# JosephCatrambone/aruco3

Hardware: NVIDIA B200
Metric: frames_per_sec_1080p_batch256 (higher is better)
Workload: dtype u8/u32 integer pixels, f32/f64 decode

## Files before the change

aruco3_b200/csrc/k3_contours.cu:

```cuda
#include <cooperative_groups.h>
#include <cooperative_groups/scan.h>
#include <cub/device/device_radix_sort.cuh>

#include <stdio.h>
#include <stdlib.h>

#include <algorithm>
#include <optional>

#include "a3_internal.h"

namespace a3 {
namespace {

namespace cg = cooperative_groups;

constexpr int kDx[8] = {-1, -1, 0, 1, 1, 1, 0, -1};
constexpr int kDy[8] = {0, -1, -1, -1, 0, 1, 1, 1};

struct StepTables {
    uint16_t fwd[8][512];
    uint16_t bwd[8][512];
};

// ... 16 lines not shown
                }
                const uint16_t e = (uint16_t)(d | (((examined >> 0) & 1u) << 3) | (((examined >> 4) & 1u) << 4) | ((kDx[d] + 1) << 5) |
                                              ((kDy[d] + 1) << 7) | (((d + 4) & 7) << 10));
                (back ? t.bwd : t.fwd)[state][hood] = e;
            }
        }
}

__device__ __forceinline__ int ddx(int d) { return (d >= 3 && d <= 5) ? 1 : ((d == 2 || d == 6) ? 0 : -1); }
__device__ __forceinline__ int ddy(int d) { return (d >= 1 && d <= 3) ? -1 : ((d == 0 || d == 4) ? 0 : 1); }

struct Geo {
    const uint32_t *planes;
    uint32_t n, w, h, wpr, Hp;
    size_t frame_words;
};

__device__ __forceinline__ uint32_t hood9(const uint32_t *plane, uint32_t Hp, int x, int y) {
    const int o = x + 31;
    const uint32_t *p = plane + ((uint32_t)(o >> 5) * Hp + (uint32_t)y);
    const int sh = o & 31;
    uint32_t t = __ldg(p) >> sh, m = __ldg(p + 1) >> sh, b = __ldg(p + 2) >> sh;
    if (sh > 29) {
        const uint32_t *q = p + Hp;
        t |= __ldg(q) << (32 - sh); m |= __ldg(q + 1) << (32 - sh); b |= __ldg(q + 2) << (32 - sh);
    }
    return (t & 7u) | ((m & 7u) << 3) | ((b & 7u) << 6);
}
__device__ __forceinline__ uint32_t ring_of(uint32_t hood) {
    const uint32_t t = hood & 7u, m = (hood >> 3) & 7u, b = hood >> 6;
    return (m & 1u) | ((t & 1u) << 1) | ((t & 2u) << 1) | ((t & 4u) << 1) | ((m & 4u) << 2) | ((b & 4u) << 3) | ((b & 2u) << 5) | ((b & 1u) << 7);
}

struct Window {
    const uint32_t *plane;
    uint32_t Hp;
    int kc, yg;
    uint32_t t, m, b;
    uint32_t t2, m2, b2;
    uint32_t v2;
};
__device__ __forceinline__ void win_load(Window &w, int x, int y) {
    w.kc = (x + 31) >> 5; w.yg = y;
    const uint32_t *p = w.plane + (size_t)w.kc * w.Hp + y;
    w.t = __ldg(p); w.m = __ldg(p + 1); w.b = __ldg(p + 2);
    w.v2 = 0;
}
__device__ __forceinline__ uint32_t win_hood(Window &w, int x) {
    const int sh = (x + 31) & 31;
    uint32_t t = w.t >> sh, m = w.m >> sh, b = w.b >> sh;
    if (sh > 29) {
        if (w.v2 != 7u) {
            const uint32_t *q = w.plane + (size_t)(w.kc + 1) * w.Hp + w.yg;
            if (!(w.v2 & 1u)) w.t2 = __ldg(q);
            if (!(w.v2 & 2u)) w.m2 = __ldg(q + 1);
            if (!(w.v2 & 4u)) w.b2 = __ldg(q + 2);
            w.v2 = 7u;
        }
        t |= w.t2 << (32 - sh); m |= w.m2 << (32 - sh); b |= w.b2 << (32 - sh);
    }
    return (t & 7u) | ((m & 7u) << 3) | ((b & 7u) << 6);
}
__device__ __forceinline__ void win_move(Window &w, int x, int y) {
    const int kc = (x + 31) >> 5, dy = y - w.yg;
    if (kc != w.kc) {
        if (dy == 0 && kc == w.kc + 1 && w.v2 == 7u) {
            w.t = w.t2; w.m = w.m2; w.b = w.b2; w.v2 = 0; w.kc = kc;
        } else if (dy == 0 && kc == w.kc - 1) {
            w.t2 = w.t; w.m2 = w.m; w.b2 = w.b; w.v2 = 7u; w.kc = kc;
            const uint32_t *p = w.plane + (size_t)kc * w.Hp + y;
            w.t = __ldg(p); w.m = __ldg(p + 1); w.b = __ldg(p + 2);
        } else {
            win_load(w, x, y);
        }
    } else if (dy > 0) {
        w.t = w.m; w.m = w.b; w.b = __ldg(w.plane + (size_t)kc * w.Hp + y + 2);
        w.t2 = w.m2; w.m2 = w.b2; w.v2 >>= 1;
        w.yg = y;
    } else if (dy < 0) {
        w.b = w.m; w.m = w.t; w.t = __ldg(w.plane + (size_t)kc * w.Hp + y);
        w.b2 = w.m2; w.m2 = w.t2; w.v2 = (w.v2 << 1) & 7u;
        w.yg = y;
    }
}

constexpr uint32_t kBudget = 48;
constexpr uint32_t kSeg = 64;
static_assert(kBudget < kSeg, "borders finished inside the budget must fit one emit segment");
struct Ckpt { uint32_t walker, pos, xy, state; };
constexpr uint32_t kCkptBackward = 0x80000000u;

enum { kDead = 0, kSurvivor = 1, kUndecided = 2 };
constexpr uint32_t kNumWalkers = 0;
constexpr uint32_t kNumLong = 1;
constexpr uint32_t kOverflow = 2;
constexpr uint32_t kNumCands = 3;
constexpr uint32_t kNumCkpts = 4;
constexpr uint32_t kSpecFail = 5;
constexpr uint32_t kNumRelays = 6;
constexpr uint32_t kMaxFrameLong = 7;

struct Lists {
    unsigned long long *cands;
    uint32_t cands_cap;
    unsigned long long *walkers;
    unsigned long long *long_keys;
    uint32_t *long_n;
    uint32_t *counters;
    uint32_t *long_slot;
    uint32_t *walker_slot;
    Ckpt *ckpts;
    uint32_t ckpt_cap;
    unsigned long long *long_points;
    uint32_t walkers_cap, long_cap;
    uint32_t *frame_contours;
    unsigned long long *frame_points;
    uint32_t *frame_flags;
    uint32_t *long_off_slot;
    uint32_t frame_cap;
    uint32_t *frame_long_count;
    unsigned long long *frame_keys;
    uint32_t *frame_slots;
    uint2 *relays;
    struct Seg *segs;
    uint32_t *relay_base;
    unsigned long long *seg_owner;
    struct Jump *jumps;
    unsigned long long *anchor_owner;
    uint32_t jump_hops;
    uint32_t relay_cap;
    uint32_t relay_shift, nrr;
};
struct __align__(16) Seg {
    uint32_t next;
    uint32_t len;
    uint32_t cand;
    uint32_t cand_pos;
    uint32_t min_pix;
    uint32_t slot;
    uint32_t off;
    uint32_t state;
};
struct __align__(16) Jump {
    uint32_t dest;
    uint32_t len;
    uint32_t cand;
    uint32_t cand_off;
    uint32_t min_pix;
    uint32_t min_idx;
    uint32_t pad0, pad1;
};
constexpr uint32_t kNone = 0xffffffffu;
constexpr uint32_t kRelayFlag = 0x80000000u;


__device__ __forceinline__ uint32_t hood2(const uint32_t *plane, uint32_t Hp, int o, int y) {
    const uint32_t *p = plane + ((uint32_t)(o >> 5) * Hp + (uint32_t)y);
    const int sh = o & 31;
    uint32_t t = __ldg(p), m = __ldg(p + 1), b = __ldg(p + 2), t2 = 0, m2 = 0, b2 = 0;
    if (sh > 29) {
        const uint32_t *q = p + Hp;
        t2 = __ldg(q); m2 = __ldg(q + 1); b2 = __ldg(q + 2);
    }
    t = __funnelshift_r(t, t2, sh); m = __funnelshift_r(m, m2, sh); b = __funnelshift_r(b, b2, sh);
    return ((t << 1) & 0x00eu) | ((m << 4) & 0x070u) | ((b << 7) & 0x380u);
}

template <bool relay_on>
__device__ int walk_border(const uint32_t *plane, const Geo &g, const uint16_t (*fwd)[512], const uint16_t (*bwd)[512], int sx, int sy, int kind,
                           uint32_t budget, uint32_t &n, bool &first_pixel, uint32_t rmask) {
    const int w = (int)g.w, o_max = w + 30;
    const uint32_t start_pix = (uint32_t)(sy * w + sx);
    const uint32_t me = (start_pix << 1) | (uint32_t)kind;
    const uint32_t nb0 = ring_of(hood9(plane, g.Hp, sx, sy));
    const int adj = kind ? 4 : 0;
    int pred = -1;
    for (int k = 0; k < 8; k++) {
        const int d = (adj + k) & 7;
        if ((nb0 >> d) & 1) { pred = d; break; }
    }
    n = 1;
    first_pixel = true;
    if (pred < 0) return (kind == 0 || sx == 0) ? kSurvivor : kDead;
    if (relay_on && ((uint32_t)sy & rmask) == 0u) return kDead;
    uint32_t min_pix = start_pix, pix = start_pix, state_off;
    int o = sx + 31, y = sy;
    if (kind) {
        state_off = (uint32_t)pred << 10;
        n = 0;
    } else {
        o += ddx(pred); y += ddy(pred); pix = (uint32_t)(y * w + o - 31); state_off = (uint32_t)((pred + 4) & 7) << 10;
    }
    const unsigned char *lut = reinterpret_cast<const unsigned char *>(kind ? &fwd[0][0] : &bwd[0][0]);
    const uint32_t tw = (me + 1u) >> 1, te = me >> 1, pred_off = (uint32_t)pred << 10;
    for (uint32_t steps = 0;; steps++) {
        const uint32_t e = *reinterpret_cast<const uint16_t *>(lut + state_off + hood2(plane, g.Hp, o, y));
        if (kind) {
            if (n && pix == start_pix && state_off == pred_off) break;
        } else {
            if (pix == start_pix && (e & 8u)) break;
        }
        if (relay_on && ((uint32_t)y & rmask) == 0u && (((e & 8u) && o > 31) || ((e & 16u) && o < o_max))) return kDead;
        if ((e & 8u) && o > 31 && pix < tw) return kDead;
        if ((e & 16u) && o < o_max && pix < te) return kDead;
        if (steps >= budget) return kUndecided;
        min_pix = min(min_pix, pix);
        n++;
        const int dx = (int)((e >> 5) & 3u) - 1, dy = (int)((e >> 7) & 3u) - 1;
        o += dx; y += dy;
        pix += (uint32_t)(dy * w + dx);
        state_off = e & 0x1c00u;
    }
    first_pixel = min_pix == start_pix;
    return kSurvivor;
}

__device__ __forceinline__ uint32_t record_survivor(const Lists &l, uint32_t frame, unsigned long long key, int kind, uint32_t n, bool first_pixel,
                                                    uint32_t min_points, bool relay = false) {
    atomicAdd(&l.frame_contours[frame], 1u);
    atomicAdd(&l.frame_points[frame], (unsigned long long)n);
    if (kind == 0 && !first_pixel) atomicOr(&l.frame_flags[frame], 1u);
    if (n >= min_points && n >= 4) {
        const uint32_t slot = atomicAdd(&l.counters[kNumLong], 1u);
        if (slot < l.long_cap) {
            l.long_keys[slot] = key;
            l.long_n[slot] = relay ? (n | kRelayFlag) : n;
            l.long_slot[slot] = slot;
            l.long_off_slot[slot] = (uint32_t)atomicAdd(l.long_points, (unsigned long long)n);
            if (l.frame_cap) {
                const uint32_t j = atomicAdd(&l.frame_long_count[frame], 1u);
                if (j < l.frame_cap) {
                    l.frame_keys[(size_t)frame * l.frame_cap + j] = key;
                    l.frame_slots[(size_t)frame * l.frame_cap + j] = slot;
                }
                atomicMax(&l.counters[kMaxFrameLong], j + 1);
            }
            return slot;
        }
        atomicOr(&l.counters[kOverflow], 1u);
    }
    return 0xffffffffu;
}

template <bool RELAY>
__global__ void __launch_bounds__(256) k3_candidates(const Geo g, const StepTables *tables, const uint32_t min_points, const Lists l) {
    __shared__ uint16_t fwd[8][512];
    __shared__ uint16_t bwd[8][512];
    for (int i = threadIdx.x; i < 8 * 512; i += blockDim.x) {
        (&fwd[0][0])[i] = (&tables->fwd[0][0])[i];
        (&bwd[0][0])[i] = (&tables->bwd[0][0])[i];
    }
    __syncthreads();
    const uint32_t words_per_frame = g.h * g.wpr;
    constexpr int kBatch = 4;
    const uint32_t stride = blockDim.x;
    const uint32_t last_k = (g.w - 1) >> 5, last_bit = (g.w - 1) & 31;
    for (uint32_t frame = blockIdx.y; frame < g.n; frame += gridDim.y)
    for (uint32_t k = blockIdx.x; k < g.wpr; k += gridDim.x)
    for (uint32_t base0 = blockIdx.z * stride * kBatch; base0 < g.h; base0 += gridDim.z * stride * kBatch) {
// ... 312 lines not shown
    const uint32_t rmask = (1u << l.relay_shift) - 1u;
    for (uint32_t i = tid >> 1; i < total; i += (gridDim.x * blockDim.x) >> 1) {
        const unsigned long long key = l.walkers[i];
        uint32_t frame;
        int sx, sy, kind;
        decode_key(g, key, frame, sx, sy, kind);
        const uint32_t *plane = g.planes + (size_t)frame * g.frame_words;
        asm volatile("" : "+l"(plane));
        const uint32_t start_pix = (uint32_t)(sy * w + sx);
        const uint32_t me = (start_pix << 1) | (uint32_t)kind;
        const uint32_t nb0 = ring_of(hood9(plane, g.Hp, sx, sy));
        const int adj = kind ? 4 : 0;
        int pred = -1;
        for (int k = 0; k < 8; k++) {
            const int d = (adj + k) & 7;
            if ((nb0 >> d) & 1) { pred = d; break; }
        }
        if (pred < 0) {
            if (!back) {
                uint32_t slot = 0xffffffffu;
                if (kind == 0 || sx == 0) slot = record_survivor(l, frame, key, kind, 1, true, min_points);
                l.walker_slot[i] = slot;
            }
            continue;
        }
        int o = sx + 31, y = sy;
        uint32_t pix = start_pix, state_off = (uint32_t)pred << 10;
        if (back) {
            o += ddx(pred); y += ddy(pred); pix = (uint32_t)(y * w + o - 31); state_off = (uint32_t)((pred + 4) & 7) << 10;
        }
        const uint32_t tw = (me + 1u) >> 1, te = me >> 1;
        uint32_t min_pix = start_pix, n = 0, prev_back_id = 0xffffffffu, my_prev_id = 0xffffffffu;
        bool dead = false;
        uint32_t meet_id = 0;
        for (uint32_t s0 = 0;; s0 += kBlk) {
            uint32_t ids[kBlk];
            bool mine_dead = false;
#pragma unroll
            for (int k = 0; k < kBlk; k++) {
                const uint32_t h2 = hood2(plane, g.Hp, o, y);
                const uint32_t e = *reinterpret_cast<const uint16_t *>(lut + state_off + h2);
                const uint32_t fstate = back ? (e & 7u) : (state_off >> 10);
                ids[k] = (pix << 3) | fstate;
                mine_dead |= ((e & 8u) && o > 31 && pix < tw) || ((e & 16u) && o < o_max && pix < te) ||
                             (relay_on && ((uint32_t)y & rmask) == 0u && (((e & 8u) && o > 31) || ((e & 16u) && o < o_max)));
                min_pix = min(min_pix, pix);
                const uint32_t walked = back ? s0 + k + 1 : s0 + k;
                if (walked && walked % kSeg == 0) {
                    const uint32_t c = atomicAdd(&l.counters[kNumCkpts], 1u);
                    if (c < l.ckpt_cap) l.ckpts[c] = Ckpt{i, walked, (uint32_t)(o - 31) | ((uint32_t)y << 16), fstate | (back ? kCkptBackward : 0u)};
                    else atomicOr(&l.counters[kOverflow], 1u);
                }
                const int dx = (int)((e >> 5) & 3u) - 1, dy = (int)((e >> 7) & 3u) - 1;
                o += dx; y += dy;
                pix += (uint32_t)(dy * w + dx);
                state_off = e & 0x1c00u;
            }
            uint32_t oid[kBlk];
#pragma unroll
            for (int k = 0; k < kBlk; k++) oid[k] = __shfl_xor_sync(pair_mask, ids[k], 1);
            dead = __shfl_xor_sync(pair_mask, (int)mine_dead, 1) || mine_dead;
            if (dead) break;
            bool met = false;
#pragma unroll
            for (int k = 0; k < kBlk; k++) {
                if (met) continue;
                const uint32_t s = s0 + k;
                const uint32_t fwd_id = back ? oid[k] : ids[k], back_id = back ? ids[k] : oid[k];
                const uint32_t back_prev = k == 0 ? (back ? my_prev_id : prev_back_id) : (back ? ids[k > 0 ? k - 1 : 0] : oid[k > 0 ? k - 1 : 0]);
                if (fwd_id == back_id) { n = 2 * s + 1; met = true; meet_id = ids[k]; }
                else if (s > 0 && fwd_id == back_prev) { n = 2 * s; met = true; meet_id = ids[k]; }
            }
            if (met) break;
            my_prev_id = ids[kBlk - 1];
            prev_back_id = oid[kBlk - 1];
        }
        min_pix = min(min_pix, __shfl_xor_sync(pair_mask, min_pix, 1));
        if (back) continue;
        uint32_t slot = 0xffffffffu;
        if (!dead) {
            if (n > kSeg) {
                const uint32_t c = atomicAdd(&l.counters[kNumCkpts], 1u);
                const uint32_t mp = meet_id >> 3, my = mp / (uint32_t)w, mx = mp - my * (uint32_t)w;
                if (c < l.ckpt_cap) l.ckpts[c] = Ckpt{i, n / 2, mx | (my << 16), meet_id & 7u};
                else atomicOr(&l.counters[kOverflow], 1u);
            }
            slot = record_survivor(l, frame, key, kind, n, min_pix == start_pix, min_points);
        }
        l.walker_slot[i] = slot;
    }
}

__global__ void __launch_bounds__(256) k3_rank(const uint32_t *slot_sorted, const uint32_t *long_n, const uint32_t *off_slot, uint32_t n_long,
                                               uint32_t *n_sorted, uint32_t *off_sorted, uint32_t *rank) {
    const uint32_t ci = blockIdx.x * blockDim.x + threadIdx.x;
    if (ci >= n_long) return;
    const uint32_t s = slot_sorted[ci];
    if (s == 0xffffffffu) {
        n_sorted[ci] = 0;
        off_sorted[ci] = 0;
        return;
    }
    n_sorted[ci] = long_n[s];
    off_sorted[ci] = off_slot[s];
    rank[s] = ci;
}

constexpr uint32_t kOrderCap = 1024;
__global__ void __launch_bounds__(256) k3_order(const Lists l, uint32_t n_frames, unsigned long long *keys_sorted, uint32_t *n_sorted,
                                                uint32_t *off_sorted, uint32_t *rank, const uint32_t *dyn) {
    __shared__ unsigned long long keys[kOrderCap];
    __shared__ uint32_t partial[8];
    if (dyn && dyn[kSpecFail]) return;
    const uint32_t f = blockIdx.x, cap = l.frame_cap;
    uint32_t before = 0;
    for (uint32_t i = threadIdx.x; i < f; i += blockDim.x) before += min(l.frame_long_count[i], cap);
    for (int o = 16; o; o >>= 1) before += __shfl_xor_sync(0xffffffffu, before, o);
    if ((threadIdx.x & 31) == 0) partial[threadIdx.x >> 5] = before;
    const uint32_t m = min(l.frame_long_count[f], cap);
    const unsigned long long *fk = l.frame_keys + (size_t)f * cap;
    for (uint32_t i = threadIdx.x; i < m; i += blockDim.x) keys[i] = fk[i];
// ... 1 lines not shown
    uint32_t base = 0;
    for (uint32_t i = 0; i < blockDim.x / 32; i++) base += partial[i];
    for (uint32_t i = threadIdx.x; i < m; i += blockDim.x) {
        const unsigned long long k = keys[i];
        uint32_t r = 0;
        for (uint32_t j = 0; j < m; j++) r += keys[j] < k ? 1u : 0u;
        const uint32_t ci = base + r, slot = l.frame_slots[(size_t)f * cap + i];
        keys_sorted[ci] = k;
        n_sorted[ci] = l.long_n[slot];
        off_sorted[ci] = l.long_off_slot[slot];
        rank[slot] = ci;
    }
}

__global__ void __launch_bounds__(256) k3_spec_prepare(unsigned long long *long_keys, uint32_t *long_slot, uint32_t *counters,
                                                       const unsigned long long *long_points, uint32_t cap_long, uint32_t cap_ckpts,
                                                       unsigned long long cap_points, uint32_t cap_frame_long, uint32_t cap_relays) {
    const uint32_t i = blockIdx.x * blockDim.x + threadIdx.x;
    const uint32_t n_long = counters[kNumLong];
    if (i == 0)
        counters[kSpecFail] = (counters[kOverflow] || n_long > cap_long || counters[kNumCkpts] > cap_ckpts || *long_points > cap_points ||
                               counters[kMaxFrameLong] > cap_frame_long || counters[kNumRelays] > cap_relays) ? 1u : 0u;
    if (i >= n_long && i < cap_long) {
        long_keys[i] = ~0ull;
        long_slot[i] = 0xffffffffu;
    }
}

struct Contour {
    uint32_t frame, start, n, kind;
    unsigned long long point_off;
};

template <bool LIGHT>
__global__ void __launch_bounds__(128) k3_emit(const Geo g, const StepTables *tables, const unsigned long long *keys, const uint32_t *lens,
                                               const uint32_t *offsets, uint32_t n_contours, const uint32_t *rank, const uint32_t *walker_slot,
                                               const Ckpt *ckpts, uint32_t n_ckpts, Contour *contours, uint32_t *points, const uint32_t *dyn,
                                               const uint2 *relays, const Seg *segs, const unsigned long long *seg_owner, uint32_t n_relays) {
    __shared__ uint16_t fwd[8][512];
    if (dyn) {
        if (dyn[kSpecFail]) return;
        n_contours = dyn[kNumLong]; n_ckpts = dyn[kNumCkpts]; n_relays = min(n_relays, dyn[kNumRelays]);
        if (blockIdx.x * blockDim.x >= n_contours + n_ckpts + n_relays) return;
    }
    for (int i = threadIdx.x; i < 8 * 512; i += blockDim.x) (&fwd[0][0])[i] = (&tables->fwd[0][0])[i];
    __syncthreads();
    const uint32_t t = blockIdx.x * blockDim.x + threadIdx.x;
    if (t >= n_contours + n_ckpts + n_relays) return;
    uint32_t frame, ci, first, count, state;
    int x, y, sx, sy, kind;
    if (t >= n_contours + n_ckpts) {
        const uint32_t ri = t - n_contours - n_ckpts;
        const Seg sg = segs[ri];
        if (sg.len == 0) return;
        const unsigned long long own = seg_owner[ri];
        const uint32_t leader = (uint32_t)(own >> 32), cum = (uint32_t)own;
        const uint32_t slot = segs[leader].slot, start = segs[leader].off;
        if (slot == kNone) return;
        const uint2 r = relays[ri];
        ci = rank[slot];
        const uint32_t n = lens[ci] & ~kRelayFlag;
        uint32_t *out = points + offsets[ci];
        const uint32_t *plane = g.planes + (size_t)(r.y >> 1) * g.frame_words;
        asm volatile("" : "+l"(plane));
        const unsigned char *lut = reinterpret_cast<const unsigned char *>(&fwd[0][0]);
        int o = (int)(r.x & 0xffffu) + 31, yy = (int)(r.x >> 16);
        uint32_t state_off = sg.state << 10, pos = cum >= start ? cum - start : cum + n - start;
        for (uint32_t i = 0; i < sg.len; i++) {
            out[pos] = (uint32_t)(o - 31) | ((uint32_t)yy << 16);
            if (++pos == n) pos = 0;
            const uint32_t e = *reinterpret_cast<const uint16_t *>(lut + state_off + hood2(plane, g.Hp, o, yy));
            o += (int)((e >> 5) & 3u) - 1;
            yy += (int)((e >> 7) & 3u) - 1;
            state_off = e & 0x1c00u;
        }
        return;
    }
    if (t < n_contours) {
        ci = t;
        decode_key(g, keys[ci], frame, sx, sy, kind);
        const uint32_t *plane = g.planes + (size_t)frame * g.frame_words;
        const uint32_t nb0 = ring_of(hood9(plane, g.Hp, sx, sy));
        const int adj = kind ? 4 : 0;
        int pred = 0;
        for (int q = 0; q < 8; q++) {
            const int d = (adj + q) & 7;
            if ((nb0 >> d) & 1) { pred = d; break; }
        }
        const uint32_t n = lens[ci] & ~kRelayFlag;
        first = 0; count = (lens[ci] & kRelayFlag) ? 0u : min(kSeg, n);
        x = sx; y = sy; state = (uint32_t)pred;
        Contour c;
        c.frame = frame; c.start = (uint32_t)sx | ((uint32_t)sy << 16); c.n = n; c.kind = (uint32_t)kind; c.point_off = offsets[ci];
        contours[ci] = c;
    } else {
        const Ckpt c = ckpts[t - n_contours];
        const uint32_t slot = walker_slot[c.walker];
        if (slot == 0xffffffffu) return;
        ci = rank[slot];
        decode_key(g, keys[ci], frame, sx, sy, kind);
        const uint32_t n = lens[ci] & ~kRelayFlag;
        first = (c.state & kCkptBackward) ? n - c.pos : c.pos;
        count = min(kSeg, n - first);
        x = (int)(c.xy & 0xffffu); y = (int)(c.xy >> 16); state = c.state & 7u;
    }
    Window win;
    win.plane = g.planes + (size_t)frame * g.frame_words; win.Hp = g.Hp;
    if constexpr (!LIGHT) win_load(win, x, y);
    uint32_t *out = points + offsets[ci] + first;
    uint32_t i = 0;
    const uint32_t *plane = win.plane;
    asm volatile("" : "+l"(plane));
    const unsigned char *lut = reinterpret_cast<const unsigned char *>(&fwd[0][0]);
    int o = x + 31;
    uint32_t state_off = state << 10;
    auto step = [&]() {
        if constexpr (LIGHT) {
            const uint32_t v = (uint32_t)(o - 31) | ((uint32_t)y << 16);
            const uint32_t e = *reinterpret_cast<const uint16_t *>(lut + state_off + hood2(plane, g.Hp, o, y));
            o += (int)((e >> 5) & 3u) - 1;
            y += (int)((e >> 7) & 3u) - 1;
            state_off = e & 0x1c00u;
            return v;
        } else {
            const uint32_t v = (uint32_t)x | ((uint32_t)y << 16);
            const uint32_t e = fwd[state][win_hood(win, x)];
            x += (int)((e >> 5) & 3u) - 1;
            y += (int)((e >> 7) & 3u) - 1;
            state = e >> 10;
            win_move(win, x, y);
            return v;
        }
    };
    while (i < count && ((uintptr_t)(out + i) & 15u)) out[i++] = step();
    for (; i + 4 <= count; i += 4) {
        uint4 v;
        v.x = step(); v.y = step(); v.z = step(); v.w = step();
        *reinterpret_cast<uint4 *>(out + i) = v;
    }
    while (i < count) out[i++] = step();
}

struct Pt { int x, y; };
__device__ __forceinline__ Pt unpack(uint32_t v) { return Pt{(int)(v & 0xffffu), (int)(v >> 16)}; }

__device__ __forceinline__ int orient(Pt p, Pt q, Pt r) {
    const long long v = (long long)(q.y - p.y) * (r.x - q.x) - (long long)(q.x - p.x) * (r.y - q.y);
    return v == 0 ? 0 : (v > 0 ? 1 : -1);
}
__device__ __forceinline__ double pdist(Pt p, Pt q) {
    const double dx = (double)p.x - (double)q.x, dy = (double)p.y - (double)q.y;
    return sqrt(dx * dx + dy * dy);
}
__device__ bool hull4(Pt q[4]) {
    int sp = 0;
    for (int i = 1; i < 4; i++)
        if (q[i].y < q[sp].y || (q[i].y == q[sp].y && q[i].x < q[sp].x)) sp = i;
    const Pt start = q[sp];
    Pt tmp[4] = {q[0], q[1], q[2], q[3]};
    { const Pt t = tmp[0]; tmp[0] = tmp[sp]; tmp[sp] = t; }
    Pt rest[3] = {tmp[1], tmp[2], tmp[3]};
    for (int i = 1; i < 3; i++) {
        const Pt key = rest[i];
        int j = i;
        while (j > 0) {
            const int o = orient(start, key, rest[j - 1]);
            const bool less = o == 0 ? pdist(start, key) < pdist(start, rest[j - 1]) : o < 0;
            if (!less) break;
            rest[j] = rest[j - 1];
            j--;
        }
        rest[j] = key;
    }
// ... 245 lines not shown
    }
    __syncwarp();
    if (lane == 0) {
        uint32_t kept = 0;
        for (uint32_t i = 0; i < nq; i++)
            if (!dead[i]) {
                for (int c = 0; c < 8; c++) dst[(size_t)kept * 8 + c] = sq[(size_t)i * 8 + c];
                kept++;
            }
        out_counts[f] = kept;
    }
}

}

namespace {
struct ListSizes {
    uint32_t n_long = 0, ckpts = 0, relays = 0, frame_long = 0;
    unsigned long long points = 0;
    bool overflow = false;
    bool fits(const ListSizes &cap) const {
        return !overflow && n_long <= cap.n_long && ckpts <= cap.ckpts && points <= cap.points && frame_long <= cap.frame_long &&
               relays <= cap.relays;
    }
};
}

struct K3Workspace::Impl {
    DevBuf<StepTables> tables;
    DevBuf<unsigned long long> cands, walkers, long_keys, long_keys_sorted, long_points, frame_points, frame_keys, seg_owner, anchor_owner;
    DevBuf<uint32_t> counters, walker_slot, long_n, long_n_sorted, long_off, long_slot, long_slot_sorted, long_rank, long_off_slot;
    DevBuf<uint32_t> frame_contours, frame_long_count, frame_slots, relay_base;
    DevBuf<Ckpt> ckpts;
    DevBuf<uint2> relays;
    DevBuf<Seg> segs;
    DevBuf<Jump> jumps;
    DevBuf<uint8_t> cub_tmp;
    DevBuf<Contour> contours;
    DevBuf<uint32_t> contour_quads, points;
    DevBuf<uint8_t> dead;
    PinBuf<unsigned long long> h_counts;
    Geo g;
    Lists l;
    struct History {
        uint32_t n = 0, w = 0, h = 0;
        ListSizes sizes;
        bool valid = false;
    } hist;
    std::optional<ListSizes> spec;
};

K3Workspace::K3Workspace() : impl(new Impl()) {}
K3Workspace::~K3Workspace() = default;

#define K3_CUDA(expr)                              \
    do {                                           \
        cudaError_t e__ = (expr);                  \
        if (e__ != cudaSuccess) return e__;        \
    } while (0)

static __global__ void k3_flag_all(uint32_t *frame_flags, uint32_t n, const uint32_t *counters, int force) {
    const uint32_t i = blockIdx.x * blockDim.x + threadIdx.x;
    if (i < n && (force || counters[kOverflow])) frame_flags[i] |= 8u;
}

struct PhaseTimer {
// ... 28 lines not shown

cudaError_t k3_begin(K3Workspace &ws, const K3Params &p, cudaStream_t stream) {
    K3Workspace::Impl &w = *ws.impl;
    if (p.n == 0) return cudaSuccess;
    PhaseTimer timer(stream);
    if (p.w > 65535 || p.h > 65535) return cudaErrorInvalidValue;
    if ((unsigned long long)p.w * p.h >= (1ull << 29)) return cudaErrorInvalidValue;
    Geo g;
    g.planes = p.planes; g.n = p.n; g.w = p.w; g.h = p.h; g.wpr = (p.w + 31) / 32; g.Hp = p.h + 2;
    g.frame_words = (size_t)(g.wpr + 2) * g.Hp;
    if (!w.tables.p) {
        StepTables *t = new StepTables();
        build_tables(*t);
        cudaError_t e = w.tables.reserve(1);
        if (e == cudaSuccess) e = cudaMemcpy(w.tables.p, t, sizeof(StepTables), cudaMemcpyHostToDevice);
        delete t;
        K3_CUDA(e);
        K3_CUDA(w.h_counts.reserve(8));
        K3_CUDA(w.counters.reserve(8));
        K3_CUDA(w.long_points.reserve(1));
    }
    const size_t pixels = (size_t)p.w * p.h;
    const size_t mp = p.min_points < 4 ? 4 : p.min_points;
    const size_t want_walkers = (size_t)p.n * (pixels / 32 + 4096), want_long = (size_t)p.n * (pixels / (4 * mp) + 1024);
    size_t want_cands = (size_t)p.n * (pixels / 8 + 4096);
    {
        const size_t roomy = (size_t)p.n * (pixels / 3), cap = (size_t)16 << 20;
        const size_t alt = roomy < cap ? roomy : cap;
        if (alt > want_cands) want_cands = alt;
    }
    K3_CUDA(w.cands.reserve(want_cands));
    K3_CUDA(w.walkers.reserve(want_walkers));
    K3_CUDA(w.walker_slot.reserve(want_walkers));
    const size_t want_ckpts = (size_t)p.n * (pixels / kSeg + 4096);
    K3_CUDA(w.ckpts.reserve(want_ckpts));
    if (want_long > w.long_keys.cap) {
        for (DevBuf<uint32_t> *b : {&w.long_n, &w.long_n_sorted, &w.long_off, &w.long_slot, &w.long_slot_sorted, &w.long_rank, &w.long_off_slot})
            K3_CUDA(b->reserve(want_long));
        K3_CUDA(w.long_keys_sorted.reserve(want_long));
        size_t need = 0;
        K3_CUDA(cub::DeviceRadixSort::SortPairs(nullptr, need, w.long_keys.p, w.long_keys_sorted.p, w.long_slot.p, w.long_slot_sorted.p, (int)want_long, 0, 64, stream));
        K3_CUDA(w.cub_tmp.reserve(need));
        K3_CUDA(w.long_keys.reserve(want_long));
    }
    K3_CUDA(w.frame_points.reserve(p.n));
    K3_CUDA(w.frame_contours.reserve(p.n));
    K3_CUDA(w.frame_long_count.reserve(p.n));
    const bool frame_lists = p.n <= 4096;
    if (frame_lists) {
        K3_CUDA(w.frame_keys.reserve((size_t)p.n * kOrderCap));
        K3_CUDA(w.frame_slots.reserve((size_t)p.n * kOrderCap));
    }
    K3_CUDA(w.dead.reserve((size_t)p.n * p.quad_cap));
    const char *relay_env = getenv("A3_K3_RELAY_MAX_FRAMES");
    const bool relays_off = p.n > (relay_env ? (uint32_t)strtoul(relay_env, nullptr, 10) : 16u);
    const uint32_t relay_shift = p.h > 1200 ? 5u : 4u, nrr = (p.h + (1u << relay_shift) - 1) >> relay_shift;
    size_t want_relays = relays_off ? 0 : (size_t)p.n * nrr * (p.w / 2 + 64);
    if (want_relays > ((size_t)48 << 20)) want_relays = (size_t)48 << 20;
    if (const char *cap_env = getenv("A3_K3_RELAY_CAP")) {
        const size_t c = strtoull(cap_env, nullptr, 10);
        if (want_relays > c) want_relays = c ? c : 1;
    }
    K3_CUDA(w.relays.reserve(want_relays));
    K3_CUDA(w.segs.reserve(want_relays));
    K3_CUDA(w.seg_owner.reserve(want_relays));
    K3_CUDA(w.anchor_owner.reserve(want_relays));
    K3_CUDA(w.jumps.reserve(want_relays));
    K3_CUDA(w.relay_base.reserve(relays_off ? 0 : (size_t)p.n * nrr * ((p.w + 31) / 32)));
    K3_CUDA(cudaMemsetAsync(w.frame_points.p, 0, (size_t)p.n * 8, stream));
    K3_CUDA(cudaMemsetAsync(w.frame_contours.p, 0, (size_t)p.n * 4, stream));
    K3_CUDA(cudaMemsetAsync(w.frame_long_count.p, 0, (size_t)p.n * 4, stream));
    K3_CUDA(cudaMemsetAsync(p.frame_flags, 0, (size_t)p.n * 4, stream));
    K3_CUDA(cudaMemsetAsync(w.counters.p, 0, 32, stream));
    K3_CUDA(cudaMemsetAsync(w.long_points.p, 0, 8, stream));

    timer.mark("begin");
    Lists l;
    l.cands = w.cands.p; l.cands_cap = (uint32_t)(w.cands.cap > 0xffffffffull ? 0xffffffffull : w.cands.cap);
    l.walkers = w.walkers.p; l.long_keys = w.long_keys.p; l.long_n = w.long_n.p; l.counters = w.counters.p; l.long_points = w.long_points.p;
    l.walkers_cap = (uint32_t)(w.walkers.cap > 0xffffffffull ? 0xffffffffull : w.walkers.cap);
    l.long_cap = (uint32_t)(w.long_keys.cap > 0x7fffffffull ? 0x7fffffffull : w.long_keys.cap);
    l.frame_contours = w.frame_contours.p; l.frame_points = w.frame_points.p; l.frame_flags = p.frame_flags;
    l.long_slot = w.long_slot.p; l.walker_slot = w.walker_slot.p; l.ckpts = w.ckpts.p;
    l.long_off_slot = w.long_off_slot.p; l.frame_cap = frame_lists ? kOrderCap : 0u; l.frame_long_count = w.frame_long_count.p;
    l.frame_keys = w.frame_keys.p; l.frame_slots = w.frame_slots.p;
    l.ckpt_cap = (uint32_t)(w.ckpts.cap > 0x7fffffffull ? 0x7fffffffull : w.ckpts.cap);
    l.relays = w.relays.p; l.segs = w.segs.p; l.seg_owner = w.seg_owner.p; l.relay_base = w.relay_base.p; l.relay_cap = (uint32_t)want_relays;
    l.relay_shift = relay_shift; l.nrr = nrr;
    l.jumps = w.jumps.p; l.anchor_owner = w.anchor_owner.p;
    {
        const char *jump_env = getenv("A3_K3_JUMP");
        const unsigned long jh = jump_env ? strtoul(jump_env, nullptr, 10) : 32ul;
        l.jump_hops = jh < 1 ? 1u : (jh > 1024 ? 1024u : (uint32_t)jh);
    }
    int dev = 0, sms = 148;
    cudaGetDevice(&dev);
    cudaDeviceGetAttribute(&sms, cudaDevAttrMultiProcessorCount, dev);
    const StepTables *tables = w.tables.p;
    {
        const uint32_t resident = (uint32_t)sms * 8;
        const uint32_t gy = p.n < resident ? p.n : resident;
        uint32_t gx = (resident + gy - 1) / gy;
        if (gx > g.wpr) gx = g.wpr;
        const uint32_t passes = (p.h + 1023) / 1024;
        uint32_t bd = ((p.h + 4 * passes - 1) / (4 * passes) + 31) & ~31u;
        if (bd < 64) bd = 64;
        if (bd > 256) bd = 256;
        uint32_t gz = 1;
        if ((uint64_t)gx * gy * 2 <= resident) {
            bd = 64;
            gz = (p.h + 4 * bd - 1) / (4 * bd);
            const uint32_t room = resident / (gx * gy);
            if (gz > room) gz = room;
            if (gz < 1) gz = 1;
        }
        if (l.relay_cap) k3_candidates<true><<<dim3(gx, gy, gz), bd, 0, stream>>>(g, tables, p.min_points, l);
        else k3_candidates<false><<<dim3(gx, gy, gz), bd, 0, stream>>>(g, tables, p.min_points, l);
    }
    K3_CUDA(cudaGetLastError());
// ... 41 lines not shown
    const size_t fin_smem = (size_t)p.quad_cap * (32 + 4 + 1) + 16;
    if (fin_smem > 200 * 1024) return cudaErrorInvalidValue;
    const Geo &g = w.g;
    const Lists &l = w.l;
    const size_t words_per_frame = (size_t)g.h * g.wpr, nwords = words_per_frame * p.n;
    PhaseTimer timer(stream);
    timer.mark("begin");
    if (s.n_long) {
        if (s.n_long > w.contours.cap) {
            const size_t c = (size_t)s.n_long + s.n_long / 4 + 1024;
            K3_CUDA(w.contours.reserve(c));
            K3_CUDA(w.contour_quads.reserve(c * 8));
        }
        const size_t need = (size_t)s.points + 1;
        if (need > w.points.cap) K3_CUDA(w.points.reserve(need + need / 4 + 1024));
        if (dyn) {
            k3_spec_prepare<<<(s.n_long + 255) / 256, 256, 0, stream>>>(w.long_keys.p, w.long_slot.p, w.counters.p, w.long_points.p, s.n_long,
                                                                        s.ckpts, s.points, s.frame_long, s.relays);
            K3_CUDA(cudaGetLastError());
        }
        if (l.frame_cap && s.frame_long <= l.frame_cap) {
            k3_order<<<p.n, 256, 0, stream>>>(l, p.n, w.long_keys_sorted.p, w.long_n_sorted.p, w.long_off.p, w.long_rank.p, dyn);
            K3_CUDA(cudaGetLastError());
        } else {
            size_t tmp = w.cub_tmp.cap;
            const int end_bit = 64 - __builtin_clzll(((unsigned long long)nwords << 6) | 1ull);
            K3_CUDA(cub::DeviceRadixSort::SortPairs(w.cub_tmp.p, tmp, w.long_keys.p, w.long_keys_sorted.p, w.long_slot.p, w.long_slot_sorted.p,
                                                    (int)s.n_long, 0, end_bit, stream));
            k3_rank<<<(s.n_long + 255) / 256, 256, 0, stream>>>(w.long_slot_sorted.p, w.long_n.p, w.long_off_slot.p, s.n_long, w.long_n_sorted.p,
                                                               w.long_off.p, w.long_rank.p);
            K3_CUDA(cudaGetLastError());
        }
        timer.mark("order");
        (p.n <= 4 ? k3_emit<true> : k3_emit<false>)<<<(s.n_long + s.ckpts + s.relays + 127) / 128, 128, 0, stream>>>(
            g, w.tables.p, w.long_keys_sorted.p, w.long_n_sorted.p, w.long_off.p, s.n_long, w.long_rank.p, w.walker_slot.p, w.ckpts.p, s.ckpts,
            w.contours.p, w.points.p, dyn, w.relays.p, w.segs.p, w.seg_owner.p, s.relays);
        K3_CUDA(cudaGetLastError());
        timer.mark("emit");
        k3_rdp<<<(s.n_long + 3) / 4, 128, 0, stream>>>(w.contours.p, w.points.p, s.n_long, p.eps_factor, p.min_edge_length, w.contour_quads.p,
                                                        p.frame_flags, dyn, p.w <= 16384 && p.h <= 16384);
        K3_CUDA(cudaGetLastError());
    }
    timer.mark("rdp");
    K3_CUDA(cudaFuncSetAttribute(k3_finalize, cudaFuncAttributeMaxDynamicSharedMemorySize, (int)fin_smem));
    k3_finalize<<<p.n, 32, fin_smem, stream>>>(w.contour_quads.p, w.long_keys_sorted.p, words_per_frame, s.n_long, p.n, p.min_corner_separation,
                                               p.quad_cap, p.quads, p.quad_counts, p.before_discard, p.frame_flags, w.dead.p, dyn);
    K3_CUDA(cudaGetLastError());
    timer.mark("finalize");
    if (p.frame_contours) K3_CUDA(cudaMemcpyAsync(p.frame_contours, w.frame_contours.p, (size_t)p.n * 4, cudaMemcpyDeviceToDevice, stream));
    if (p.frame_points) K3_CUDA(cudaMemcpyAsync(p.frame_points, w.frame_points.p, (size_t)p.n * 8, cudaMemcpyDeviceToDevice, stream));
    return cudaSuccess;
}

cudaError_t k3_finish(K3Workspace &ws, const K3Params &p, cudaStream_t stream) {
    K3Workspace::Impl &w = *ws.impl;
    if (p.n == 0) return cudaSuccess;
    K3_CUDA(cudaStreamSynchronize(stream));
    const ListSizes s = read_sizes(w);
    if (getenv("A3_K3_TIMING")) {
        const uint32_t *hc = reinterpret_cast<const uint32_t *>(w.h_counts.p);
        fprintf(stderr, "k3 lists: %u candidates, %u walkers, %u long borders, %llu points, %u checkpoints, %u relay cracks\n", hc[kNumCands],
                hc[kNumWalkers], s.n_long, s.points, s.ckpts, s.relays);
    }
    record_history(w, p, s);
    w.spec.reset();
    const bool wide = s.points >= 0xffffffffull;
    if (wide && !s.overflow) {
        k3_flag_all<<<(p.n + 127) / 128, 128, 0, stream>>>(p.frame_flags, p.n, w.counters.p, 1);
        K3_CUDA(cudaGetLastError());
// ... 43 lines not shown
```

Baseline: 201,200.

## Stash walked border ids in a pool so emit copies instead of re-tracing

The paired walker kernel now writes each block of traced pixel ids into a global pool indexed by checkpoint, with one checkpoint per 64-step segment. The emit kernel copies these segments warp-cooperatively, reversing backward halves, instead of re-walking the border from checkpoints. The Window-based re-trace and the LIGHT template are removed. Re-walking is kept only as a fallback when the pool overflows. This trades extra global writes in the walk phase and up to 256MB of pool memory for cheaper emit, and it adds per-segment atomics plus more complex checkpoint bookkeeping.

```diff
diff --git a/aruco3_b200/csrc/k3_contours.cu b/aruco3_b200/csrc/k3_contours.cu
--- a/aruco3_b200/csrc/k3_contours.cu
+++ b/aruco3_b200/csrc/k3_contours.cu
@@ -72,63 +72,10 @@
     return (m & 1u) | ((t & 1u) << 1) | ((t & 2u) << 1) | ((t & 4u) << 1) | ((m & 4u) << 2) | ((b & 4u) << 3) | ((b & 2u) << 5) | ((b & 1u) << 7);
 }
 
-struct Window {
-    const uint32_t *plane;
-    uint32_t Hp;
-    int kc, yg;
-    uint32_t t, m, b;
-    uint32_t t2, m2, b2;
-    uint32_t v2;
-};
-__device__ __forceinline__ void win_load(Window &w, int x, int y) {
-    w.kc = (x + 31) >> 5; w.yg = y;
-    const uint32_t *p = w.plane + (size_t)w.kc * w.Hp + y;
-    w.t = __ldg(p); w.m = __ldg(p + 1); w.b = __ldg(p + 2);
-    w.v2 = 0;
-}
-__device__ __forceinline__ uint32_t win_hood(Window &w, int x) {
-    const int sh = (x + 31) & 31;
-    uint32_t t = w.t >> sh, m = w.m >> sh, b = w.b >> sh;
-    if (sh > 29) {
-        if (w.v2 != 7u) {
-            const uint32_t *q = w.plane + (size_t)(w.kc + 1) * w.Hp + w.yg;
-            if (!(w.v2 & 1u)) w.t2 = __ldg(q);
-            if (!(w.v2 & 2u)) w.m2 = __ldg(q + 1);
-            if (!(w.v2 & 4u)) w.b2 = __ldg(q + 2);
-            w.v2 = 7u;
-        }
-        t |= w.t2 << (32 - sh); m |= w.m2 << (32 - sh); b |= w.b2 << (32 - sh);
-    }
-    return (t & 7u) | ((m & 7u) << 3) | ((b & 7u) << 6);
-}
-__device__ __forceinline__ void win_move(Window &w, int x, int y) {
-    const int kc = (x + 31) >> 5, dy = y - w.yg;
-    if (kc != w.kc) {
-        if (dy == 0 && kc == w.kc + 1 && w.v2 == 7u) {
-            w.t = w.t2; w.m = w.m2; w.b = w.b2; w.v2 = 0; w.kc = kc;
-        } else if (dy == 0 && kc == w.kc - 1) {
-            w.t2 = w.t; w.m2 = w.m; w.b2 = w.b; w.v2 = 7u; w.kc = kc;
-            const uint32_t *p = w.plane + (size_t)kc * w.Hp + y;
-            w.t = __ldg(p); w.m = __ldg(p + 1); w.b = __ldg(p + 2);
-        } else {
-            win_load(w, x, y);
-        }
-    } else if (dy > 0) {
-        w.t = w.m; w.m = w.b; w.b = __ldg(w.plane + (size_t)kc * w.Hp + y + 2);
-        w.t2 = w.m2; w.m2 = w.b2; w.v2 >>= 1;
-        w.yg = y;
-    } else if (dy < 0) {
-        w.b = w.m; w.m = w.t; w.t = __ldg(w.plane + (size_t)kc * w.Hp + y);
-        w.b2 = w.m2; w.m2 = w.t2; w.v2 = (w.v2 << 1) & 7u;
-        w.yg = y;
-    }
-}
-
 constexpr uint32_t kBudget = 48;
 constexpr uint32_t kSeg = 64;
-static_assert(kBudget < kSeg, "borders finished inside the budget must fit one emit segment");
-struct Ckpt { uint32_t walker, pos, xy, state; };
-constexpr uint32_t kCkptBackward = 0x80000000u;
+struct Ckpt { uint32_t walker, blk, id; };
+constexpr uint32_t kCkptBackward = 0x80000000u, kCkptMeet = 0x40000000u;
 
 enum { kDead = 0, kSurvivor = 1, kUndecided = 2 };
 constexpr uint32_t kNumWalkers = 0;
@@ -151,6 +98,8 @@
     uint32_t *walker_slot;
     Ckpt *ckpts;
     uint32_t ckpt_cap;
+    uint32_t *pool;
+    uint32_t pool_blocks;
     unsigned long long *long_points;
     uint32_t walkers_cap, long_cap;
     uint32_t *frame_contours;
@@ -191,7 +140,7 @@
     uint32_t pad0, pad1;
 };
 constexpr uint32_t kNone = 0xffffffffu;
-constexpr uint32_t kRelayFlag = 0x80000000u;
+constexpr uint32_t kSegmented = 0x80000000u;
 
 
 __device__ __forceinline__ uint32_t hood2(const uint32_t *plane, uint32_t Hp, int o, int y) {
@@ -256,7 +205,7 @@
 }
 
 __device__ __forceinline__ uint32_t record_survivor(const Lists &l, uint32_t frame, unsigned long long key, int kind, uint32_t n, bool first_pixel,
-                                                    uint32_t min_points, bool relay = false) {
+                                                    uint32_t min_points, bool segmented = false) {
     atomicAdd(&l.frame_contours[frame], 1u);
     atomicAdd(&l.frame_points[frame], (unsigned long long)n);
     if (kind == 0 && !first_pixel) atomicOr(&l.frame_flags[frame], 1u);
@@ -264,7 +213,7 @@
         const uint32_t slot = atomicAdd(&l.counters[kNumLong], 1u);
         if (slot < l.long_cap) {
             l.long_keys[slot] = key;
-            l.long_n[slot] = relay ? (n | kRelayFlag) : n;
+            l.long_n[slot] = segmented ? (n | kSegmented) : n;
             l.long_slot[slot] = slot;
             l.long_off_slot[slot] = (uint32_t)atomicAdd(l.long_points, (unsigned long long)n);
             if (l.frame_cap) {
@@ -643,8 +592,10 @@
         const uint32_t tw = (me + 1u) >> 1, te = me >> 1;
         uint32_t min_pix = start_pix, n = 0, prev_back_id = 0xffffffffu, my_prev_id = 0xffffffffu;
         bool dead = false;
-        uint32_t meet_id = 0;
-        for (uint32_t s0 = 0;; s0 += kBlk) {
+        static_assert(kBlk % 4 == 0 && kSeg % kBlk == 0, "a block of steps is whole 16-byte stores inside one pool block");
+        uint32_t meet_id = 0, s0 = 0, c = kNone;
+        for (;; s0 += kBlk) {
+            if (s0 % kSeg == 0) c = atomicAdd(&l.counters[kNumCkpts], 1u);
             uint32_t ids[kBlk];
             bool mine_dead = false;
 #pragma unroll
@@ -656,12 +607,6 @@
                 mine_dead |= ((e & 8u) && o > 31 && pix < tw) || ((e & 16u) && o < o_max && pix < te) ||
                              (relay_on && ((uint32_t)y & rmask) == 0u && (((e & 8u) && o > 31) || ((e & 16u) && o < o_max)));
                 min_pix = min(min_pix, pix);
-                const uint32_t walked = back ? s0 + k + 1 : s0 + k;
-                if (walked && walked % kSeg == 0) {
-                    const uint32_t c = atomicAdd(&l.counters[kNumCkpts], 1u);
-                    if (c < l.ckpt_cap) l.ckpts[c] = Ckpt{i, walked, (uint32_t)(o - 31) | ((uint32_t)y << 16), fstate | (back ? kCkptBackward : 0u)};
-                    else atomicOr(&l.counters[kOverflow], 1u);
-                }
                 const int dx = (int)((e >> 5) & 3u) - 1, dy = (int)((e >> 7) & 3u) - 1;
                 o += dx; y += dy;
                 pix += (uint32_t)(dy * w + dx);
@@ -670,8 +615,18 @@
             uint32_t oid[kBlk];
 #pragma unroll
             for (int k = 0; k < kBlk; k++) oid[k] = __shfl_xor_sync(pair_mask, ids[k], 1);
+            if (s0 % kSeg == 0) {
+                if (c < l.ckpt_cap) l.ckpts[c] = Ckpt{i, (s0 / kSeg) | (back ? kCkptBackward | kCkptMeet : 0u), ids[0]};
+                else atomicOr(&l.counters[kOverflow], 1u);
+            }
             dead = __shfl_xor_sync(pair_mask, (int)mine_dead, 1) || mine_dead;
             if (dead) break;
+            if (c < l.pool_blocks) {
+                uint4 *b = reinterpret_cast<uint4 *>(l.pool + (size_t)c * kSeg + s0 % kSeg);
+#pragma unroll
+                for (int k = 0; k < kBlk; k += 4) b[k / 4] = make_uint4(ids[k], ids[k + 1], ids[k + 2], ids[k + 3]);
+            }
+            if (back && (s0 + kBlk) % kSeg == 0 && c < l.ckpt_cap) l.ckpts[c] = Ckpt{i, (s0 / kSeg) | kCkptBackward, ids[kBlk - 1]};
             bool met = false;
 #pragma unroll
             for (int k = 0; k < kBlk; k++) {
@@ -687,17 +642,12 @@
             prev_back_id = oid[kBlk - 1];
         }
         min_pix = min(min_pix, __shfl_xor_sync(pair_mask, min_pix, 1));
-        if (back) continue;
-        uint32_t slot = 0xffffffffu;
-        if (!dead) {
-            if (n > kSeg) {
-                const uint32_t c = atomicAdd(&l.counters[kNumCkpts], 1u);
-                const uint32_t mp = meet_id >> 3, my = mp / (uint32_t)w, mx = mp - my * (uint32_t)w;
-                if (c < l.ckpt_cap) l.ckpts[c] = Ckpt{i, n / 2, mx | (my << 16), meet_id & 7u};
-                else atomicOr(&l.counters[kOverflow], 1u);
-            }
-            slot = record_survivor(l, frame, key, kind, n, min_pix == start_pix, min_points);
-        }
+        const uint32_t fwd_meet = __shfl_xor_sync(pair_mask, meet_id, 1);
+        if (back) {
+            if (!dead && (s0 + kBlk) % kSeg != 0 && c < l.ckpt_cap) l.ckpts[c] = Ckpt{i, (s0 / kSeg) | kCkptBackward | kCkptMeet, fwd_meet};
+            continue;
+        }
+        const uint32_t slot = dead ? kNone : record_survivor(l, frame, key, kind, n, min_pix == start_pix, min_points, true);
         l.walker_slot[i] = slot;
     }
 }
@@ -765,11 +715,11 @@
     unsigned long long point_off;
 };
 
-template <bool LIGHT>
 __global__ void __launch_bounds__(128) k3_emit(const Geo g, const StepTables *tables, const unsigned long long *keys, const uint32_t *lens,
                                                const uint32_t *offsets, uint32_t n_contours, const uint32_t *rank, const uint32_t *walker_slot,
-                                               const Ckpt *ckpts, uint32_t n_ckpts, Contour *contours, uint32_t *points, const uint32_t *dyn,
-                                               const uint2 *relays, const Seg *segs, const unsigned long long *seg_owner, uint32_t n_relays) {
+                                               const Ckpt *ckpts, uint32_t n_ckpts, const uint32_t *pool, uint32_t pool_blocks, Contour *contours,
+                                               uint32_t *points, const uint32_t *dyn, const uint2 *relays, const Seg *segs,
+                                               const unsigned long long *seg_owner, uint32_t n_relays) {
     __shared__ uint16_t fwd[8][512];
     if (dyn) {
         if (dyn[kSpecFail]) return;
@@ -778,100 +728,128 @@
     }
     for (int i = threadIdx.x; i < 8 * 512; i += blockDim.x) (&fwd[0][0])[i] = (&tables->fwd[0][0])[i];
     __syncthreads();
+    const unsigned char *lut = reinterpret_cast<const unsigned char *>(&fwd[0][0]);
     const uint32_t t = blockIdx.x * blockDim.x + threadIdx.x;
-    if (t >= n_contours + n_ckpts + n_relays) return;
-    uint32_t frame, ci, first, count, state;
-    int x, y, sx, sy, kind;
-    if (t >= n_contours + n_ckpts) {
+    uint32_t frame = 0, steps = 0, skip = 0, state_off = 0, copy = 0, blk = 0, dst = 0;
+    bool reversed = false;
+    int o = 0, y = 0;
+    uint32_t *out = points;
+    if (t >= n_contours + n_ckpts + n_relays) {
+    } else if (t >= n_contours + n_ckpts) {
         const uint32_t ri = t - n_contours - n_ckpts;
         const Seg sg = segs[ri];
-        if (sg.len == 0) return;
         const unsigned long long own = seg_owner[ri];
         const uint32_t leader = (uint32_t)(own >> 32), cum = (uint32_t)own;
-        const uint32_t slot = segs[leader].slot, start = segs[leader].off;
-        if (slot == kNone) return;
-        const uint2 r = relays[ri];
-        ci = rank[slot];
-        const uint32_t n = lens[ci] & ~kRelayFlag;
-        uint32_t *out = points + offsets[ci];
-        const uint32_t *plane = g.planes + (size_t)(r.y >> 1) * g.frame_words;
-        asm volatile("" : "+l"(plane));
-        const unsigned char *lut = reinterpret_cast<const unsigned char *>(&fwd[0][0]);
-        int o = (int)(r.x & 0xffffu) + 31, yy = (int)(r.x >> 16);
-        uint32_t state_off = sg.state << 10, pos = cum >= start ? cum - start : cum + n - start;
-        for (uint32_t i = 0; i < sg.len; i++) {
-            out[pos] = (uint32_t)(o - 31) | ((uint32_t)yy << 16);
-            if (++pos == n) pos = 0;
-            const uint32_t e = *reinterpret_cast<const uint16_t *>(lut + state_off + hood2(plane, g.Hp, o, yy));
-            o += (int)((e >> 5) & 3u) - 1;
-            yy += (int)((e >> 7) & 3u) - 1;
-            state_off = e & 0x1c00u;
-        }
-        return;
-    }
-    if (t < n_contours) {
-        ci = t;
+        const uint32_t slot = sg.len ? segs[leader].slot : kNone, start = sg.len ? segs[leader].off : 0;
+        if (slot != kNone) {
+            const uint2 r = relays[ri];
+            const uint32_t ci = rank[slot];
+            const uint32_t n = lens[ci] & ~kSegmented;
+            uint32_t *seg_out = points + offsets[ci];
+            const uint32_t *plane = g.planes + (size_t)(r.y >> 1) * g.frame_words;
+            asm volatile("" : "+l"(plane));
+            int so = (int)(r.x & 0xffffu) + 31, yy = (int)(r.x >> 16);
+            uint32_t sst = sg.state << 10, pos = cum >= start ? cum - start : cum + n - start;
+            for (uint32_t i = 0; i < sg.len; i++) {
+                seg_out[pos] = (uint32_t)(so - 31) | ((uint32_t)yy << 16);
+                if (++pos == n) pos = 0;
+                const uint32_t e = *reinterpret_cast<const uint16_t *>(lut + sst + hood2(plane, g.Hp, so, yy));
+                so += (int)((e >> 5) & 3u) - 1;
+                yy += (int)((e >> 7) & 3u) - 1;
+                sst = e & 0x1c00u;
+            }
+        }
+    } else if (t < n_contours) {
+        const uint32_t ci = t;
+        int sx, sy, kind;
         decode_key(g, keys[ci], frame, sx, sy, kind);
-        const uint32_t *plane = g.planes + (size_t)frame * g.frame_words;
-        const uint32_t nb0 = ring_of(hood9(plane, g.Hp, sx, sy));
-        const int adj = kind ? 4 : 0;
-        int pred = 0;
-        for (int q = 0; q < 8; q++) {
-            const int d = (adj + q) & 7;
-            if ((nb0 >> d) & 1) { pred = d; break; }
-        }
-        const uint32_t n = lens[ci] & ~kRelayFlag;
-        first = 0; count = (lens[ci] & kRelayFlag) ? 0u : min(kSeg, n);
-        x = sx; y = sy; state = (uint32_t)pred;
+        const uint32_t n = lens[ci] & ~kSegmented;
         Contour c;
         c.frame = frame; c.start = (uint32_t)sx | ((uint32_t)sy << 16); c.n = n; c.kind = (uint32_t)kind; c.point_off = offsets[ci];
         contours[ci] = c;
+        if (!(lens[ci] & kSegmented)) {
+            const uint32_t nb0 = ring_of(hood9(g.planes + (size_t)frame * g.frame_words, g.Hp, sx, sy));
+            const int adj = kind ? 4 : 0;
+            int pred = 0;
+            for (int q = 0; q < 8; q++) {
+                const int d = (adj + q) & 7;
+                if ((nb0 >> d) & 1) { pred = d; break; }
+            }
+            o = sx + 31; y = sy; state_off = (uint32_t)pred << 10; steps = n;
+            out = points + offsets[ci];
+        }
     } else {
-        const Ckpt c = ckpts[t - n_contours];
-        const uint32_t slot = walker_slot[c.walker];
-        if (slot == 0xffffffffu) return;
-        ci = rank[slot];
-        decode_key(g, keys[ci], frame, sx, sy, kind);
-        const uint32_t n = lens[ci] & ~kRelayFlag;
-        first = (c.state & kCkptBackward) ? n - c.pos : c.pos;
-        count = min(kSeg, n - first);
-        x = (int)(c.xy & 0xffffu); y = (int)(c.xy >> 16); state = c.state & 7u;
-    }
-    Window win;
-    win.plane = g.planes + (size_t)frame * g.frame_words; win.Hp = g.Hp;
-    if constexpr (!LIGHT) win_load(win, x, y);
-    uint32_t *out = points + offsets[ci] + first;
-    uint32_t i = 0;
-    const uint32_t *plane = win.plane;
-    asm volatile("" : "+l"(plane));
-    const unsigned char *lut = reinterpret_cast<const unsigned char *>(&fwd[0][0]);
-    int o = x + 31;
-    uint32_t state_off = state << 10;
-    auto step = [&]() {
-        if constexpr (LIGHT) {
-            const uint32_t v = (uint32_t)(o - 31) | ((uint32_t)y << 16);
+        const uint32_t ri = t - n_contours;
+        const Ckpt r = ckpts[ri];
+        const uint32_t slot = walker_slot[r.walker];
+        if (slot != kNone) {
+            const uint32_t ci = rank[slot];
+            const uint32_t n = lens[ci] & ~kSegmented, half = n - n / 2, j = r.blk & ~(kCkptBackward | kCkptMeet);
+            uint32_t lo, hi, from;
+            reversed = (r.blk & kCkptBackward) != 0;
+            if (reversed) {
+                hi = n - j * kSeg;
+                lo = hi >= half + kSeg ? hi - kSeg : half;
+                from = (r.blk & kCkptMeet) ? n / 2 : hi - kSeg;
+            } else {
+                lo = j * kSeg;
+                hi = min(lo + kSeg, half);
+                from = lo;
+            }
+            if (lo < hi) {
+                if (ri < pool_blocks) {
+                    copy = hi - lo; blk = ri; dst = offsets[ci] + lo;
+                } else {
+                    int sx, sy, kind;
+                    decode_key(g, keys[ci], frame, sx, sy, kind);
+                    const uint32_t pix = r.id >> 3, py = pix / g.w;
+                    o = (int)(pix - py * g.w) + 31; y = (int)py; state_off = (r.id & 7u) << 10;
+                    steps = hi - from; skip = lo - from;
+                    out = points + offsets[ci] + lo;
+                }
+            }
+        }
+    }
+    if (steps) {
+        const uint32_t *plane = g.planes + (size_t)frame * g.frame_words;
+        asm volatile("" : "+l"(plane));
+        for (uint32_t i = 0; i < steps; i++) {
             const uint32_t e = *reinterpret_cast<const uint16_t *>(lut + state_off + hood2(plane, g.Hp, o, y));
+            if (i >= skip) out[i - skip] = (uint32_t)(o - 31) | ((uint32_t)y << 16);
             o += (int)((e >> 5) & 3u) - 1;
             y += (int)((e >> 7) & 3u) - 1;
             state_off = e & 0x1c00u;
-            return v;
-        } else {
-            const uint32_t v = (uint32_t)x | ((uint32_t)y << 16);
-            const uint32_t e = fwd[state][win_hood(win, x)];
-            x += (int)((e >> 5) & 3u) - 1;
-            y += (int)((e >> 7) & 3u) - 1;
-            state = e >> 10;
-            win_move(win, x, y);
-            return v;
-        }
-    };
-    while (i < count && ((uintptr_t)(out + i) & 15u)) out[i++] = step();
-    for (; i + 4 <= count; i += 4) {
-        uint4 v;
-        v.x = step(); v.y = step(); v.z = step(); v.w = step();
-        *reinterpret_cast<uint4 *>(out + i) = v;
-    }
-    while (i < count) out[i++] = step();
+        }
+    }
+    static_assert(kSeg == 64, "two points per lane and record");
+    const int lane = threadIdx.x & 31;
+    for (uint32_t pending = __ballot_sync(0xffffffffu, copy != 0); pending;) {
+        constexpr int kGroup = 4;
+        uint32_t cnt[kGroup], d[kGroup], v[kGroup][2];
+#pragma unroll
+        for (int u = 0; u < kGroup; u++) {
+            const int src = pending ? __ffs(pending) - 1 : 0;
+            cnt[u] = __shfl_sync(0xffffffffu, copy, src);
+            d[u] = __shfl_sync(0xffffffffu, dst, src);
+            const uint32_t b = __shfl_sync(0xffffffffu, blk, src);
+            const bool rev = __shfl_sync(0xffffffffu, reversed, src);
+            if (!pending) cnt[u] = 0;
+            pending &= pending - 1;
+            const uint32_t *in = pool + (size_t)b * kSeg;
+#pragma unroll
+            for (int h = 0; h < 2; h++) {
+                const uint32_t m = (uint32_t)lane + 32u * h;
+                v[u][h] = m < cnt[u] ? in[rev ? cnt[u] - 1 - m : m] : 0u;
+            }
+        }
+#pragma unroll
+        for (int u = 0; u < kGroup; u++)
+#pragma unroll
+            for (int h = 0; h < 2; h++) {
+                const uint32_t m = (uint32_t)lane + 32u * h, pix = v[u][h] >> 3, py = pix / g.w;
+                if (m < cnt[u]) points[d[u] + m] = (pix - py * g.w) | (py << 16);
+            }
+    }
 }
 
 struct Pt { int x, y; };
@@ -1183,6 +1161,7 @@
     DevBuf<uint32_t> counters, walker_slot, long_n, long_n_sorted, long_off, long_slot, long_slot_sorted, long_rank, long_off_slot;
     DevBuf<uint32_t> frame_contours, frame_long_count, frame_slots, relay_base;
     DevBuf<Ckpt> ckpts;
+    DevBuf<uint32_t> pool;
     DevBuf<uint2> relays;
     DevBuf<Seg> segs;
     DevBuf<Jump> jumps;
@@ -1277,8 +1256,14 @@
     K3_CUDA(w.cands.reserve(want_cands));
     K3_CUDA(w.walkers.reserve(want_walkers));
     K3_CUDA(w.walker_slot.reserve(want_walkers));
-    const size_t want_ckpts = (size_t)p.n * (pixels / kSeg + 4096);
+    const size_t want_ckpts = (size_t)p.n * (pixels / kSeg + 4096) + 2 * want_walkers;
     K3_CUDA(w.ckpts.reserve(want_ckpts));
+    size_t pool_blocks = std::min(want_ckpts, ((size_t)256 << 20) / (kSeg * sizeof(uint32_t)));
+    if (const char *pool_env = getenv("A3_K3_POOL_BLOCKS")) {
+        const size_t c = strtoull(pool_env, nullptr, 10);
+        if (pool_blocks > c) pool_blocks = c;
+    }
+    K3_CUDA(w.pool.reserve(pool_blocks * kSeg));
     if (want_long > w.long_keys.cap) {
         for (DevBuf<uint32_t> *b : {&w.long_n, &w.long_n_sorted, &w.long_off, &w.long_slot, &w.long_slot_sorted, &w.long_rank, &w.long_off_slot})
             K3_CUDA(b->reserve(want_long));
@@ -1330,6 +1315,7 @@
     l.long_off_slot = w.long_off_slot.p; l.frame_cap = frame_lists ? kOrderCap : 0u; l.frame_long_count = w.frame_long_count.p;
     l.frame_keys = w.frame_keys.p; l.frame_slots = w.frame_slots.p;
     l.ckpt_cap = (uint32_t)(w.ckpts.cap > 0x7fffffffull ? 0x7fffffffull : w.ckpts.cap);
+    l.pool = w.pool.p; l.pool_blocks = (uint32_t)std::min<size_t>(pool_blocks, l.ckpt_cap);
     l.relays = w.relays.p; l.segs = w.segs.p; l.seg_owner = w.seg_owner.p; l.relay_base = w.relay_base.p; l.relay_cap = (uint32_t)want_relays;
     l.relay_shift = relay_shift; l.nrr = nrr;
     l.jumps = w.jumps.p; l.anchor_owner = w.anchor_owner.p;
@@ -1437,9 +1423,9 @@
             K3_CUDA(cudaGetLastError());
         }
         timer.mark("order");
-        (p.n <= 4 ? k3_emit<true> : k3_emit<false>)<<<(s.n_long + s.ckpts + s.relays + 127) / 128, 128, 0, stream>>>(
+        k3_emit<<<(s.n_long + s.ckpts + s.relays + 127) / 128, 128, 0, stream>>>(
             g, w.tables.p, w.long_keys_sorted.p, w.long_n_sorted.p, w.long_off.p, s.n_long, w.long_rank.p, w.walker_slot.p, w.ckpts.p, s.ckpts,
-            w.contours.p, w.points.p, dyn, w.relays.p, w.segs.p, w.seg_owner.p, s.relays);
+            w.pool.p, l.pool_blocks, w.contours.p, w.points.p, dyn, w.relays.p, w.segs.p, w.seg_owner.p, s.relays);
         K3_CUDA(cudaGetLastError());
         timer.mark("emit");
         k3_rdp<<<(s.n_long + 3) / 4, 128, 0, stream>>>(w.contours.p, w.points.p, s.n_long, p.eps_factor, p.min_edge_length, w.contour_quads.p,
```

Measured after the change: 205,900 (median of 6 runs). 1.02x the previous value.
